# scienceguyrob/PulsarFeatureExtractor

Measured on AMD Instinct MI355X. Metric: candidates/sec (8-feature path, 128-bin), higher is better.
Workload: dtype u8->int64/f64; 1 GPU; config 2: 10000000 synthetic candidates per GPU, 128-bin profile + 128-bin DM, 8 Lyon moment features (pfe_lyon8_u8); candidates_per_gpu=10000000, dm_bins=128, parallelism=candidate shards x1, no collective

## Files before the change

### pulsarfeatureextractor_amd/csrc/lyon8.hip

```cpp

#include "options.h"
#include "pfe_common.h"

namespace pfe {

typedef short short2v __attribute__((ext_vector_type(2)));
typedef unsigned short ushort2v __attribute__((ext_vector_type(2)));
typedef uint32_t u32x4 __attribute__((ext_vector_type(4)));
typedef double f64x2 __attribute__((ext_vector_type(2)));

struct Moments {
  double mean, m2, m3, m4;
};

__device__ __forceinline__ Moments moments_i64(long long n, long long T1, long long T2,
                                               long long T3, unsigned long long T4) {
  typedef unsigned long long u64;
  const u64 un = (u64)n, t1 = (u64)T1, t2 = (u64)T2, t3 = (u64)T3;
  const u64 n2 = un * un, n3 = n2 * un;
  const u64 t1s = t1 * t1;
  const long long N2 = (long long)(un * t2 - t1s);
  const long long N3 = (long long)(n2 * t3 - 3ull * un * t1 * t2 + 2ull * t1s * t1);
  const u64 N4 = n3 * T4 - 4ull * n2 * t1 * t3 + 6ull * un * t1s * t2 - 3ull * t1s * t1s;
  const double dn = (double)n;
  Moments m;
  m.mean = (double)(T1 + 128ll * n) / dn;
  m.m2 = (double)N2 / (dn * dn);
  m.m3 = (double)N3 / (dn * dn * dn);
  m.m4 = (double)N4 / ((dn * dn) * (dn * dn));
  return m;
}

__device__ __forceinline__ double i128_to_f64(__int128 v) {
  const bool neg = v < 0;
  unsigned __int128 u = neg ? (unsigned __int128)(-v) : (unsigned __int128)v;
  const uint64_t hi = (uint64_t)(u >> 64), lo = (uint64_t)u;
  double r = (double)hi * 18446744073709551616.0 + (double)lo;
  return neg ? -r : r;
}

__device__ __forceinline__ Moments moments_i128(long long n, long long T1, long long T2,
                                                long long T3, unsigned long long T4) {
  typedef __int128 i128;
  const i128 in = n, t1 = T1, t2 = T2, t3 = T3, t4 = (i128)T4;
  const i128 n2 = in * in, n3 = n2 * in;
  const i128 t1s = t1 * t1;
  const i128 N2 = in * t2 - t1s;
  const i128 N3 = n2 * t3 - 3 * in * t1 * t2 + 2 * t1s * t1;
  const i128 N4 = n3 * t4 - 4 * n2 * t1 * t3 + 6 * in * t1s * t2 - 3 * t1s * t1s;
  const double dn = (double)n;
  Moments m;
  m.mean = (double)(T1 + 128ll * n) / dn;
  m.m2 = i128_to_f64(N2) / (dn * dn);
  m.m3 = i128_to_f64(N3) / (dn * dn * dn);
  m.m4 = i128_to_f64(N4) / ((dn * dn) * (dn * dn));
  return m;
}

__device__ __forceinline__ bool zero_var(const Moments& m) {
  const double e = 2.220446049250313e-16 * m.mean;
  return m.m2 <= e * e;
}

__device__ __forceinline__ double stat_k(const Moments& m, int k) {
  if (k == 0) return m.mean;
  if (k == 1) return sqrt(m.m2);
  if (zero_var(m)) return __builtin_nan("");
  if (k == 2) return m.m3 / (m.m2 * sqrt(m.m2));
  return m.m4 / (m.m2 * m.m2) - 3.0;
}

struct Acc2 {
  uint32_t s1, s2;
  int t3;
  uint64_t t4;
};

__device__ __forceinline__ void acc2_dword(uint32_t x, Acc2& a, uint32_t& t4a) {
  a.s1 = __builtin_amdgcn_udot4(x, 0x01010101u, a.s1, false);
  a.s2 = __builtin_amdgcn_udot4(x, x, a.s2, false);
  const uint32_t lo = __builtin_amdgcn_perm(0u, x, 0x0c020c00u);
  const uint32_t hi = __builtin_amdgcn_perm(0u, x, 0x0c030c01u);
  short2v ylo = __builtin_bit_cast(short2v, lo) - (short2v){128, 128};
  short2v yhi = __builtin_bit_cast(short2v, hi) - (short2v){128, 128};
  ushort2v qlo = __builtin_bit_cast(ushort2v, ylo) * __builtin_bit_cast(ushort2v, ylo);
  ushort2v qhi = __builtin_bit_cast(ushort2v, yhi) * __builtin_bit_cast(ushort2v, yhi);
  a.t3 = __builtin_amdgcn_sdot2(__builtin_bit_cast(short2v, qlo), ylo, a.t3, false);
  a.t3 = __builtin_amdgcn_sdot2(__builtin_bit_cast(short2v, qhi), yhi, a.t3, false);
  t4a = __builtin_amdgcn_udot2(qlo, qlo, t4a, false);
  t4a = __builtin_amdgcn_udot2(qhi, qhi, t4a, false);
}

__device__ __forceinline__ void acc2_x4(const u32x4 q, Acc2& a) {
  uint32_t u = 0, v = 0;
  acc2_dword(q.x, a, u);
  acc2_dword(q.y, a, u);
  acc2_dword(q.z, a, v);
  acc2_dword(q.w, a, v);
  a.t4 += (uint64_t)u + (uint64_t)v;
}

template <int G>
__device__ __forceinline__ void acc2_reduce(Acc2& a) {
  a.s1 = (uint32_t)group_sum_i32<G>((int)a.s1);
  a.s2 = (uint32_t)group_sum_i32<G>((int)a.s2);
  a.t3 = group_sum_i32<G>(a.t3);
  a.t4 = group_sum_u64<G>(a.t4);
}

template <int L>
__device__ __forceinline__ void stats4(const Acc2& a, double (&st)[4]) {
  constexpr double IN1 = 1.0 / L, IN2 = IN1 * IN1, IN3 = IN2 * IN1, IN4 = IN2 * IN2;
  const long long S1 = (long long)a.s1;
  const long long T1 = S1 - 128ll * L;
  const long long T2 = (long long)a.s2 - 256ll * S1 + 16384ll * L;
  const long long T3 = a.t3;
  typedef unsigned long long u64;
  const long long N2 = (long long)L * T2 - T1 * T1;
  const long long T1s = T1 * T1;
  const long long N3 = (long long)L * L * T3 - 3ll * L * T1 * T2 + 2ll * T1s * T1;
  const u64 N4 = (u64)L * L * L * a.t4 - 4ull * (u64)L * L * (u64)(T1 * T3) +
                 6ull * (u64)L * (u64)(T1s * T2) - 3ull * (u64)T1s * (u64)T1s;
  const double mean = (double)S1 * IN1;
  const double m2 = (double)N2 * IN2;
  const double m3 = (double)N3 * IN3;
  const double m4 = (double)N4 * IN4;
  const double sd = sqrt(m2);
  const double e = 2.220446049250313e-16 * mean;
  const bool zero = m2 <= e * e;
  st[0] = mean;
  st[1] = sd;
  st[2] = zero ? __builtin_nan("") : m3 / (m2 * sd);
  st[3] = zero ? __builtin_nan("") : m4 / (m2 * m2) - 3.0;
}

template <int L, int U>
__global__ __launch_bounds__(256) void lyon8_u8_fast3(const uint8_t* __restrict__ prof,
                                                      int64_t ps,
                                                      const uint8_t* __restrict__ dm,
                                                      int64_t ds, int64_t n,
                                                      double* __restrict__ out) {
  constexpr int LPC = L / 32;
  constexpr int CPW = 64 / LPC;
  constexpr int SPL = 8 / LPC;
  const int lane = threadIdx.x & 63;
  const int sub = lane % LPC;
  const int cw = lane / LPC;
  const int j0 = sub * SPL;
  const bool is_dm = j0 >= 4;
  const int64_t wave = ((int64_t)blockIdx.x * blockDim.x + threadIdx.x) >> 6;
  const int64_t step = (int64_t)CPW * U;
  const int64_t stride = (((int64_t)gridDim.x * blockDim.x) >> 6) * step;
  for (int64_t base = wave * step; base < n; base += stride) {
    u32x4 p[U][2], d[U][2];
#pragma unroll
    for (int u = 0; u < U; ++u) {
      int64_t c = base + u * CPW + cw;
      c = c < n ? c : n - 1;
      const u32x4* pp = reinterpret_cast<const u32x4*>(prof + c * ps + sub * 32);
      const u32x4* dp = reinterpret_cast<const u32x4*>(dm + c * ds + sub * 32);
      p[u][0] = __builtin_nontemporal_load(pp);
      p[u][1] = __builtin_nontemporal_load(pp + 1);
      d[u][0] = __builtin_nontemporal_load(dp);
      d[u][1] = __builtin_nontemporal_load(dp + 1);
    }
#pragma unroll
    for (int u = 0; u < U; ++u) {
      const int64_t c = base + u * CPW + cw;
      Acc2 sp = {0, 0, 0, 0}, sd = {0, 0, 0, 0};
      acc2_x4(p[u][0], sp);
      acc2_x4(p[u][1], sp);
      acc2_x4(d[u][0], sd);
      acc2_x4(d[u][1], sd);
      acc2_reduce<LPC>(sp);
      acc2_reduce<LPC>(sd);
      Acc2 s;
      s.s1 = is_dm ? sd.s1 : sp.s1;
      s.s2 = is_dm ? sd.s2 : sp.s2;
      s.t3 = is_dm ? sd.t3 : sp.t3;
      s.t4 = is_dm ? sd.t4 : sp.t4;
      double st[4];
      stats4<L>(s, st);
      if (c < n) {
        double* o = out + c * 8 + j0;
        if constexpr (SPL == 4) {
          __builtin_nontemporal_store((f64x2){st[0], st[1]}, reinterpret_cast<f64x2*>(o));
          __builtin_nontemporal_store((f64x2){st[2], st[3]}, reinterpret_cast<f64x2*>(o) + 1);
        } else if constexpr (SPL == 2) {
          const bool hi2 = (j0 & 3) != 0;
          __builtin_nontemporal_store((f64x2){hi2 ? st[2] : st[0], hi2 ? st[3] : st[1]},
                                      reinterpret_cast<f64x2*>(o));
        } else {
          const int k = j0 & 3;
          const double v = k == 0 ? st[0] : k == 1 ? st[1] : k == 2 ? st[2] : st[3];
          __builtin_nontemporal_store(v, o);
        }
      }
    }
  }
}

__global__ __launch_bounds__(256) void lyon8_u8_generic(const uint8_t* __restrict__ prof,
                                                        int64_t ps, int lp,
                                                        const uint8_t* __restrict__ dm,
                                                        int64_t ds, int ld, int64_t n,
                                                        double* __restrict__ out) {
  const int lane = threadIdx.x & 63;
  const int64_t wave = ((int64_t)blockIdx.x * blockDim.x + threadIdx.x) >> 6;
  const int64_t nwaves = ((int64_t)gridDim.x * blockDim.x) >> 6;
  for (int64_t w = wave; w < 2 * n; w += nwaves) {
    const int64_t c = w >> 1;
    const int row = (int)(w & 1);
    const uint8_t* p = row ? dm + c * ds : prof + c * ps;
    const int len = row ? ld : lp;
    long long t1 = 0, t2 = 0, t3 = 0;
    unsigned long long t4 = 0;
    for (int i = lane; i < len; i += 64) {
      const int y = (int)p[i] - 128;
      const int y2 = y * y;
      t1 += y;
      t2 += y2;
      t3 += (long long)(y2 * y);
      t4 += (unsigned long long)((uint32_t)y2 * (uint32_t)y2);
    }
    t1 = wave_sum_i64(t1);
    t2 = wave_sum_i64(t2);
    t3 = wave_sum_i64(t3);
    t4 = (unsigned long long)wave_sum_i64((long long)t4);
    if (lane < 4) {
      const Moments m = len <= 430 ? moments_i64(len, t1, t2, t3, t4)
                                   : moments_i128(len, t1, t2, t3, t4);
      out[c * 8 + row * 4 + lane] = stat_k(m, lane);
    }
  }
}

struct LongShape {
  int ld;
  int base[2];
  int m[2];
  int l[2];
  int lanes[2];
};

__device__ __forceinline__ double leaf_sumsq(const uint64_t (&w)[16], int nwords, double mean) {
  double r[8];
#pragma unroll
  for (int k = 0; k < 16; ++k) {
#pragma unroll
    for (int j = 0; j < 8; ++j) {
      const double d = (double)(uint32_t)((w[k] >> (8 * j)) & 0xFF) - mean;
      const double sq = k < nwords ? d * d : 0.0;
      if (k == 0)
        r[j] = sq;
      else
        r[j] += sq;
    }
  }
  return ((r[0] + r[1]) + (r[2] + r[3])) + ((r[4] + r[5]) + (r[6] + r[7]));
}

template <int LP>
__global__ __launch_bounds__(256) void lyon8_u8_long(const uint8_t* __restrict__ prof,
                                                     int64_t ps,
                                                     const uint8_t* __restrict__ dm,
                                                     int64_t ds, int64_t n,
                                                     double* __restrict__ out, LongShape sh) {
  constexpr int PL = LP / 16;
  const int lane = threadIdx.x & 63;
  const int h = lane >> 5, li = lane & 31;
  const int M = sh.m[h], L = sh.l[h];
  const bool has = li < sh.lanes[h];
  const int off0 = sh.base[h] + li * L * M;
  const int nw0 = has ? M / 8 : 0;
  const int nw1 = has && L == 2 ? M / 8 : 0;
  const int64_t wave = ((int64_t)blockIdx.x * blockDim.x + threadIdx.x) >> 6;
  const int64_t nwaves = ((int64_t)gridDim.x * blockDim.x) >> 6;
  for (int64_t c = wave; c < n; c += nwaves) {
    const uint8_t* drow = dm + c * ds;
    uint64_t w0[16], w1[16];
#pragma unroll
    for (int k = 0; k < 16; ++k) {
      const int a0 = k < nw0 ? off0 + 8 * k : 0;
      const int a1 = k < nw1 ? off0 + M + 8 * k : 0;
      w0[k] = __builtin_nontemporal_load(reinterpret_cast<const uint64_t*>(drow + a0));
      w1[k] = __builtin_nontemporal_load(reinterpret_cast<const uint64_t*>(drow + a1));
    }
    const int pl = lane < PL ? lane : 0;
    const u32x4 pq = __builtin_nontemporal_load(reinterpret_cast<const u32x4*>(prof + c * ps) + pl);
#pragma unroll
    for (int k = 0; k < 16; ++k) {
      if (k >= nw0) w0[k] = 0x8080808080808080ull;
      if (k >= nw1) w1[k] = 0x8080808080808080ull;
    }
    Acc2 sd = {0, 0, 0, 0};
#pragma unroll
    for (int k = 0; k < 16; k += 2) {
      acc2_x4((u32x4){(uint32_t)w0[k], (uint32_t)(w0[k] >> 32), (uint32_t)w0[k + 1],
                      (uint32_t)(w0[k + 1] >> 32)}, sd);
      acc2_x4((u32x4){(uint32_t)w1[k], (uint32_t)(w1[k] >> 32), (uint32_t)w1[k + 1],
                      (uint32_t)(w1[k + 1] >> 32)}, sd);
    }
    const int pad = 8 * (32 - nw0 - nw1);
    Acc2 sp = {0, 0, 0, 0};
    if (lane < PL) acc2_x4(pq, sp);
    const long long S1 = wave_sum_i64((long long)sd.s1 - 128ll * pad);
    const long long S2 = wave_sum_i64((long long)sd.s2 - 16384ll * pad);
    const long long T3 = wave_sum_i64((long long)sd.t3);
    const unsigned long long T4 = (unsigned long long)wave_sum_i64((long long)sd.t4);
    sp.s1 = (uint32_t)wave_sum_i64((long long)sp.s1);
    sp.s2 = (uint32_t)wave_sum_i64((long long)sp.s2);
    sp.t3 = (int)wave_sum_i64((long long)sp.t3);
    sp.t4 = (uint64_t)wave_sum_i64((long long)sp.t4);
    const double dn = (double)sh.ld;
    const double mean = (double)S1 / dn;
    const double ssq = wave_sum_f64(leaf_sumsq(w0, nw0, mean) + leaf_sumsq(w1, nw1, mean));
    if (lane < 8) {
      double v;
      if (lane < 4) {
        double st[4];
        stats4<LP>(sp, st);
        v = lane == 0 ? st[0] : lane == 1 ? st[1] : lane == 2 ? st[2] : st[3];
      } else {
        const long long T1 = S1 - 128ll * sh.ld;
        const long long T2 = S2 - 256ll * S1 + 16384ll * sh.ld;
        const Moments mo = moments_i128(sh.ld, T1, T2, T3, T4);
        const int k = lane - 4;
        v = k == 0 ? mean : k == 1 ? sqrt(ssq / dn) : stat_k(mo, k);
      }
      __builtin_nontemporal_store(v, out + c * 8 + lane);
    }
  }
}

constexpr int DPP_ROW_ROR8 = 0x128;

template <int CTRL>
__device__ __forceinline__ uint32_t dpp_u32(uint32_t v) {
  return (uint32_t)dpp_i32<CTRL>((int)v);
}

__device__ __forceinline__ uint32_t reduce_scatter8(const uint32_t (&v)[8], int t) {
  const bool b2 = t & 4, b1 = t & 2, b0 = t & 1;
  uint32_t a[4], b[2];
#pragma unroll
  for (int k = 0; k < 4; ++k)
    a[k] = (b2 ? v[k + 4] : v[k]) + dpp_u32<DPP_ROW_HALF_MIRROR>(b2 ? v[k] : v[k + 4]);
#pragma unroll
  for (int k = 0; k < 2; ++k)
    b[k] = (b1 ? a[k + 2] : a[k]) + dpp_u32<DPP_QUAD_XOR2>(b1 ? a[k] : a[k + 2]);
  return (b0 ? b[1] : b[0]) + dpp_u32<DPP_QUAD_XOR1>(b0 ? b[0] : b[1]);
}

__device__ __forceinline__ double swap16_sum(double v) {
  const long long x = __double_as_longlong(v);
  const unsigned lo = (unsigned)x, hi = (unsigned)((unsigned long long)x >> 32);
  const auto l = __builtin_amdgcn_permlane16_swap(lo, lo, false, false);
  const auto h = __builtin_amdgcn_permlane16_swap(hi, hi, false, false);
  return __longlong_as_double((long long)(((unsigned long long)h[0] << 32) | l[0])) +
         __longlong_as_double((long long)(((unsigned long long)h[1] << 32) | l[1]));
}
__device__ __forceinline__ double swap32_sum(double v) {
  const long long x = __double_as_longlong(v);
  const unsigned lo = (unsigned)x, hi = (unsigned)((unsigned long long)x >> 32);
  const auto l = __builtin_amdgcn_permlane32_swap(lo, lo, false, false);
  const auto h = __builtin_amdgcn_permlane32_swap(hi, hi, false, false);
  return __longlong_as_double((long long)(((unsigned long long)h[0] << 32) | l[0])) +
         __longlong_as_double((long long)(((unsigned long long)h[1] << 32) | l[1]));
}

__device__ __forceinline__ double leaf_tree64(double v) {
  v += dpp_f64<DPP_ROW_ROR8>(v);
  v = swap16_sum(v);
  v = swap32_sum(v);
  v += dpp_f64<DPP_QUAD_XOR1>(v);
  v += dpp_f64<DPP_QUAD_XOR2>(v);
  v += dpp_f64<DPP_ROW_HALF_MIRROR>(v);
  return v;
}

__device__ __forceinline__ void acc34_dword(uint32_t x, int& t3, uint32_t& t4a) {
  const uint32_t lo = __builtin_amdgcn_perm(0u, x, 0x0c020c00u);
  const uint32_t hi = __builtin_amdgcn_perm(0u, x, 0x0c030c01u);
  short2v ylo = __builtin_bit_cast(short2v, lo) - (short2v){128, 128};
  short2v yhi = __builtin_bit_cast(short2v, hi) - (short2v){128, 128};
  ushort2v qlo = __builtin_bit_cast(ushort2v, ylo) * __builtin_bit_cast(ushort2v, ylo);
  ushort2v qhi = __builtin_bit_cast(ushort2v, yhi) * __builtin_bit_cast(ushort2v, yhi);
  t3 = __builtin_amdgcn_sdot2(__builtin_bit_cast(short2v, qlo), ylo, t3, false);
  t3 = __builtin_amdgcn_sdot2(__builtin_bit_cast(short2v, qhi), yhi, t3, false);
  t4a = __builtin_amdgcn_udot2(qlo, qlo, t4a, false);
  t4a = __builtin_amdgcn_udot2(qhi, qhi, t4a, false);
}

template <int LP, int NI>
__global__ __launch_bounds__(256) void lyon8_u8_pow2(const uint8_t* __restrict__ prof,
                                                     int64_t ps,
                                                     const uint8_t* __restrict__ dm,
                                                     int64_t ds, int64_t n,
                                                     double* __restrict__ out) {
  static_assert(NI == 8 || NI == 16, "ld = 8192 or 16384");
  constexpr int PL = LP / 16;
  constexpr int K = NI == 16 ? 14 : 13;
  constexpr int LD = 1 << K;
  constexpr double SCALE = 1.0 / (double)(1ll << (2 * K));
  const int lane = threadIdx.x & 63;
  const int t = lane & 7;
  const int64_t wave = ((int64_t)blockIdx.x * blockDim.x + threadIdx.x) >> 6;
  const int64_t nwaves = ((int64_t)gridDim.x * blockDim.x) >> 6;
  for (int64_t c = wave; c < n; c += nwaves) {
    const u32x4* drow = reinterpret_cast<const u32x4*>(dm + c * ds) + lane;
    u32x4 q[NI];
#pragma unroll
    for (int i = 0; i < NI; ++i) q[i] = __builtin_nontemporal_load(drow + 64 * i);
    const int pl = lane < PL ? lane : 0;
    const u32x4 pq = __builtin_nontemporal_load(reinterpret_cast<const u32x4*>(prof + c * ps) + pl);
    uint32_t A[NI], B[NI];
    uint32_t s1 = 0, s2 = 0;
    int t3 = 0;
    uint64_t t4 = 0;
#pragma unroll
    for (int i = 0; i < NI; ++i) {
      uint32_t a = __builtin_amdgcn_udot4(q[i].x, 0x01010101u, 0u, false);
      a = __builtin_amdgcn_udot4(q[i].y, 0x01010101u, a, false);
      a = __builtin_amdgcn_udot4(q[i].z, 0x01010101u, a, false);
      a = __builtin_amdgcn_udot4(q[i].w, 0x01010101u, a, false);
      uint32_t b = __builtin_amdgcn_udot4(q[i].x, q[i].x, 0u, false);
      b = __builtin_amdgcn_udot4(q[i].y, q[i].y, b, false);
      b = __builtin_amdgcn_udot4(q[i].z, q[i].z, b, false);
      b = __builtin_amdgcn_udot4(q[i].w, q[i].w, b, false);
      A[i] = a;
      B[i] = b;
      s1 += a;
      s2 += b;
      uint32_t u = 0, v = 0;
      acc34_dword(q[i].x, t3, u);
      acc34_dword(q[i].y, t3, u);
      acc34_dword(q[i].z, t3, v);
      acc34_dword(q[i].w, t3, v);
      t4 += (uint64_t)u + (uint64_t)v;
    }
    Acc2 sp = {0, 0, 0, 0};
    if (lane < PL) acc2_x4(pq, sp);
    const long long S1 = wave_sum_i64((long long)s1);
    const long long S2 = wave_sum_i64((long long)s2);
    const long long T3 = wave_sum_i64((long long)t3);
    const unsigned long long T4 = (unsigned long long)wave_sum_i64((long long)t4);
    sp.s1 = (uint32_t)wave_sum_i64((long long)sp.s1);
    sp.s2 = (uint32_t)wave_sum_i64((long long)sp.s2);
    sp.t3 = (int)wave_sum_i64((long long)sp.t3);
    sp.t4 = (uint64_t)wave_sum_i64((long long)sp.t4);
    double ssq = 0.0;
#pragma unroll
    for (int s = 0; s < NI / 8; ++s) {
      uint32_t va[8], vb[8];
#pragma unroll
      for (int k = 0; k < 8; ++k) {
        va[k] = A[8 * s + k];
        vb[k] = B[8 * s + k];
      }
      const long long la = reduce_scatter8(va, t), lb = reduce_scatter8(vb, t);
      const long long v2k = (lb << (2 * K)) - ((2 * S1 * la) << K) + 128ll * S1 * S1;
      const double chunk = leaf_tree64((double)v2k * SCALE);
      ssq = s == 0 ? chunk : ssq + chunk;
    }
    if (lane < 8) {
      double v;
      if (lane < 4) {
        double st[4];
        stats4<LP>(sp, st);
        v = lane == 0 ? st[0] : lane == 1 ? st[1] : lane == 2 ? st[2] : st[3];
      } else {
        const double dn = (double)LD;
        const long long T1 = S1 - 128ll * LD;
        const long long T2 = S2 - 256ll * S1 + 16384ll * LD;
        const Moments mo = moments_i128(LD, T1, T2, T3, T4);
        const int k = lane - 4;
        v = k == 0 ? (double)S1 / dn : k == 1 ? sqrt(ssq / dn) : stat_k(mo, k);
      }
      __builtin_nontemporal_store(v, out + c * 8 + lane);
    }
  }
}

constexpr int L8_LDS_WAVE_BYTES = 64 * 144;

__device__ __forceinline__ void wave_lds_sync() {
  __builtin_amdgcn_fence(__ATOMIC_RELEASE, "wavefront");
  __builtin_amdgcn_wave_barrier();
  __builtin_amdgcn_fence(__ATOMIC_ACQUIRE, "wavefront");
}

__host__ __device__ constexpr int lds_leaf_stride(int m) { return m + ((m / 16) % 2 == 0 ? 16 : 32); }

template <int M>
__device__ __forceinline__ double leaf_sumsq_lds(const uint8_t* img, int leaf, double mean) {
  constexpr int S = lds_leaf_stride(M);
  uint64_t w[16];
// ... 452 lines not shown
      }
      double ssq = 0.0, a3 = 0.0, a4 = 0.0;
#pragma unroll
      for (int ch = 0; ch < NCH; ++ch) {
        if (ch > 0) dm_stage<NCH>(img, q, ch, lane, full_base, stab);
        wave_lds_sync();
        double l3, l4;
        double leaf;
        if (PAIRT)
          leaf = dm_leaf_tri_pair<FPM>(img, lane, nm, sc, z, l3, l4);
        else if (G == 3 && ch == NCH - 1)
          leaf = dm_leaf_tri<FPM>(img, lane, nm, sc, z, l3, l4);
        else if (G == 2 || G == 4 || G == 8) {
          if (ch == NCH - 1)
            leaf = dm_leaf<FPM, (G == 2 || G == 4 || G == 8) ? 8 / G : 8>(img + (lane / G) * DM_S,
                                                                       (8 / G) * (lane % G), nm, sc, z, nw_last, l3, l4);
          else
            leaf = dm_leaf<FPM>(img + lane * DM_S, 0, nm, sc, z, 16, l3, l4);
        }
        else
          leaf = dm_leaf<FPM>(img + lane * DM_S, 0, nm, sc, z, ch < NCH - 1 ? 16 : nw_last, l3, l4);
        if (ch == NCH - 1) {
          const bool in = leaf_last >= 0;
          leaf = in ? leaf : 0.0;
          l3 = in ? l3 : 0.0;
          l4 = in ? l4 : 0.0;
        }
        a3 += l3;
        a4 += l4;
        const double cs = PAIR ? half_sum_f64(leaf)
                          : (ch == NCH - 1 && G == 3) ? wave_sum_tri_split_f64(leaf)
                          : (ch == NCH - 1 && sh.tri) ? wave_sum_tri_f64(leaf) : wave_sum_f64(leaf);
        ssq = ch == 0 ? cs : ssq + cs;
        wave_lds_sync();
      }
      ssq = __builtin_ldexp(ssq, 102);
      if constexpr (FPM) {
        const double s3 = __builtin_ldexp(a3, 153), s4 = __builtin_ldexp(a4, 204);
        const uint64_t b3 = (uint64_t)__double_as_longlong(PAIR ? half_sum_f64(s3) : wave_sum_f64(s3));
        const uint64_t b4 = (uint64_t)__double_as_longlong(PAIR ? half_sum_f64(s4) : wave_sum_f64(s4));
        park_u32(kT3l, (uint32_t)b3);
        park_u32(kT3h, (uint32_t)(b3 >> 32));
        park_u32(kT4l, (uint32_t)b4);
        park_u32(kT4h, (uint32_t)(b4 >> 32));
      }
      if constexpr (PAIR) {
        const double va = lane_f64(ssq, 0), vb = lane_f64(ssq, 32);
        kssq = mine ? va : mine2 ? vb : kssq;
      } else {
        kssq = mine ? ssq : kssq;
      }
    }
    if (lane < cnt) {
      Acc2 sp = {0, 0, 0, 0};
      const u32x4* pr = reinterpret_cast<const u32x4*>(prof + (base + lane) * ps);
      for (int k = 0; k < ppl; ++k) acc2_x4(__builtin_nontemporal_load(pr + k), sp);
      const long long L = sh.lp;
      const long long S1p = (long long)sp.s1;
      const long long T1p = S1p - 128ll * L;
      const long long T2p = (long long)sp.s2 - 256ll * S1p + 16384ll * L;
      const long long T3p = (long long)sp.t3;
      const uint64_t T4p = sp.t4;
      const Moments mp = moments_i64(L, T1p, T2p, T3p, T4p);
      const double sdp = sqrt(mp.m2);
      const bool zp = zero_var(mp);
      const long long D = sh.ld;
      const long long S1 = (long long)kS1;
      const double dn = (double)D;
      Moments md;
      if constexpr (FPM) {
        md.mean = (double)S1 / dn;
        md.m3 = __longlong_as_double((long long)(((uint64_t)kT3h << 32) | kT3l)) / dn;
        md.m4 = __longlong_as_double((long long)(((uint64_t)kT4h << 32) | kT4l)) / dn;
      } else {
        const long long T1 = S1 - 128ll * D;
        const long long T2 = (long long)kS2 - 256ll * S1 + 16384ll * D;
        const long long T3 = (long long)(int)kT3h * 65536ll + (long long)kT3l;
        const uint64_t T4 = ((uint64_t)kT4h << 24) + (uint64_t)kT4l;
        md = moments_i128(D, T1, T2, T3, T4);
      }
      const double m2 = kssq / dn;
      const double e = 2.220446049250313e-16 * md.mean;
      const bool zd = m2 <= e * e;
      const double sdd = sqrt(m2);
      f64x2* o = reinterpret_cast<f64x2*>(out + (base + lane) * 8);
      __builtin_nontemporal_store((f64x2){mp.mean, sdp}, o);
      __builtin_nontemporal_store(
          (f64x2){zp ? __builtin_nan("") : mp.m3 / (mp.m2 * sdp),
                  zp ? __builtin_nan("") : mp.m4 / (mp.m2 * mp.m2) - 3.0}, o + 1);
      __builtin_nontemporal_store((f64x2){md.mean, sdd}, o + 2);
      __builtin_nontemporal_store(
          (f64x2){zd ? __builtin_nan("") : md.m3 / (m2 * sdd),
                  zd ? __builtin_nan("") : md.m4 / (m2 * m2) - 3.0}, o + 3);
    }
  }
}

__global__ __launch_bounds__(256) void lyon8_f64_generic(const double* __restrict__ prof,
                                                         int64_t ps, int lp,
                                                         const double* __restrict__ dm,
                                                         int64_t ds, int ld, int64_t n,
                                                         double* __restrict__ out) {
  const int lane = threadIdx.x & 63;
  const int64_t wave = ((int64_t)blockIdx.x * blockDim.x + threadIdx.x) >> 6;
  const int64_t nwaves = ((int64_t)gridDim.x * blockDim.x) >> 6;
  for (int64_t w = wave; w < 2 * n; w += nwaves) {
    const int64_t c = w >> 1;
    const int row = (int)(w & 1);
    const double* p = row ? dm + c * ds : prof + c * ps;
    const int len = row ? ld : lp;
    double s = 0.0;
    for (int i = lane; i < len; i += 64) s += p[i];
    s = wave_sum_f64(s);
    const double mean = s / (double)len;
    double a2 = 0.0, a3 = 0.0, a4 = 0.0;
    for (int i = lane; i < len; i += 64) {
      const double d = p[i] - mean;
      const double d2 = d * d;
      a2 += d2;
      a3 += d2 * d;
      a4 += d2 * d2;
    }
    a2 = wave_sum_f64(a2);
    a3 = wave_sum_f64(a3);
    a4 = wave_sum_f64(a4);
    if (lane < 4) {
      Moments m;
      m.mean = mean;
      m.m2 = a2 / (double)len;
      m.m3 = a3 / (double)len;
      m.m4 = a4 / (double)len;
      out[c * 8 + row * 4 + lane] = stat_k(m, lane);
    }
  }
}

}

namespace pfe {

static inline int grid_for(int64_t work_waves, int cap) {
  int64_t blocks = (work_waves + 3) / 4;
  if (blocks < 1) blocks = 1;
  if (blocks > cap) blocks = cap;
  return (int)blocks;
}

static bool perfect_chunk(int len, int& m, int& leaves) {
  leaves = 1;
  while (len > 128) {
    if (len % 16) return false;
    len /= 2;
    leaves *= 2;
  }
  m = len;
  return len > 64 && len % 8 == 0;
}

static bool place_half(LongShape& sh, int h, int base, int len) {
  int m, leaves;
  if (!perfect_chunk(len, m, leaves) || leaves > 64) return false;
  sh.base[h] = base;
  sh.m[h] = m;
  sh.l[h] = leaves > 32 ? 2 : 1;
  sh.lanes[h] = leaves > 32 ? 32 : leaves;
  return true;
}

static bool long_row_shape(int ld, LongShape& sh) {
  sh.ld = ld;
  if (ld <= 256) return false;
  if (ld <= 8192) {
    return ld % 16 == 0 && place_half(sh, 0, 0, ld / 2) && place_half(sh, 1, ld / 2, ld / 2);
  }
  if (ld <= 16384) return place_half(sh, 0, 0, 8192) && place_half(sh, 1, 8192, ld - 8192);
  return false;
}

static void np_leaves(int off, int n, int depth, int* start, int* len, int* dep, int& cnt, int cap) {
  if (n <= 128) {
    if (cnt < cap) {
      start[cnt] = off;
      len[cnt] = n;
      dep[cnt] = depth;
    }
    ++cnt;
    return;
  }
  int n2 = n / 2;
  n2 -= n2 % 8;
  np_leaves(off, n2, depth + 1, start, len, dep, cnt, cap);
  np_leaves(off + n2, n - n2, depth + 1, start, len, dep, cnt, cap);
}

static bool dm_shape(int lp, int ld, DmShape& sh, int& nch) {
  if (ld <= 256 || ld > 4 * 8192 || ld % 16) return false;
  nch = (ld + 8191) / 8192;
  const int len = ld - 8192 * (nch - 1);
  int start[DM_MAX_LEAVES], lens[DM_MAX_LEAVES], dep[DM_MAX_LEAVES], cnt = 0;
  np_leaves(0, len, 0, start, lens, dep, cnt, DM_MAX_LEAVES);
  if (cnt > DM_MAX_LEAVES) return false;
  bool tri = false;
  if (cnt == 48) {
    tri = true;
    for (int i = 0; i < cnt; ++i) {
      const int b = i / 3, k = i % 3;
      tri = tri && start[i] == 264 * b + (k == 0 ? 0 : k == 1 ? 128 : 192) &&
            lens[i] == (k == 0 ? 128 : k == 1 ? 64 : 72) && dep[i] == dep[0] + (k == 0 ? 0 : 1);
    }
    if (!tri) return false;
  } else {
    if ((cnt & (cnt - 1)) != 0) return false;
    for (int i = 0; i < cnt; ++i)
      if (dep[i] != dep[0] || lens[i] % 8 || lens[i] < 64 || lens[i] > 128) return false;
  }
  sh.lp = lp;
  sh.ld = ld;
  sh.len_last = len;
  sh.leaves_last = cnt;
  sh.tri = tri ? 1 : 0;
  for (int i = 0; i < cnt; ++i) sh.start[i] = (uint16_t)start[i];
  for (int i = cnt; i <= DM_MAX_LEAVES; ++i) sh.start[i] = (uint16_t)len;
  return true;
}

template <auto K>
static int resident_blocks() {
  static int cached[64] = {};
  int dev = 0;
  if (hipGetDevice(&dev) != hipSuccess || dev < 0 || dev >= 64) return 1024;
  if (cached[dev] > 0) return cached[dev];
  int per_cu = 0, cus = 0;
  if (hipOccupancyMaxActiveBlocksPerMultiprocessor(&per_cu, reinterpret_cast<const void*>(K), 256, 0) !=
          hipSuccess ||
      hipDeviceGetAttribute(&cus, hipDeviceAttributeMultiprocessorCount, dev) != hipSuccess) {
    (void)hipGetLastError();
    return 1024;
  }
  cached[dev] = (per_cu > 0 ? per_cu : 1) * (cus > 0 ? cus : 1);
  return cached[dev];
}

#ifndef PFE_DM_FPM_MAXCH
#define PFE_DM_FPM_MAXCH 4
#endif
template <int NCH, bool FPM, int G = 1>
static void launch_dm_kernel(const uint8_t* prof, int64_t ps, const uint8_t* dm, int64_t ds,
                             int64_t n, double* out, const DmShape& sh, hipStream_t st, int cap) {
  constexpr auto K = lyon8_u8_dm<NCH, FPM, G>;
  int64_t blocks = resident_blocks<K>();
  const int64_t need = (n + 3) / 4;
  if (blocks > need) blocks = need;
  if (blocks > cap) blocks = cap;
  if (blocks < 1) blocks = 1;
  hipLaunchKernelGGL(K, dim3((unsigned)blocks), dim3(256), 0, st, prof, ps, dm, ds, n, out, sh);
}

hipError_t launch_lyon8_u8(const uint8_t* prof, int64_t ps, int lp, const uint8_t* dm,
                           int64_t ds, int ld, int64_t n, double* out, hipStream_t st,
                           const Options& o) {
  if (n <= 0) return hipSuccess;
  const bool aligned = ((uintptr_t)prof % 16 == 0) && ((uintptr_t)dm % 16 == 0) &&
                       (ps % 16 == 0) && (ds % 16 == 0) && ((uintptr_t)out % 16 == 0);
  DmShape dsh{};
  int dnch = 0;
  if (o.lyon8_dm != 1 && aligned && (lp == 64 || lp == 128 || lp == 256) && ld != 8192 &&
      ld != 16384 && dm_shape(lp, ld, dsh, dnch)) {
    const int cap = o.lyon8_blocks;
    const int G = !o.lyon8_dm_split ? 1
                  : (dsh.tri && dnch == 1 && o.lyon8_dm_split == 1) ? 32
                  : dsh.tri ? 3
                  : (dnch == 1 && dsh.leaves_last > 16 && dsh.leaves_last <= 32 && o.lyon8_dm_split == 1) ? 16
                  : dsh.leaves_last <= 8 ? 8 : dsh.leaves_last <= 16 ? 4 : dsh.leaves_last <= 32 ? 2 : 1;
    if (o.lyon8_dm == 0 && dnch <= PFE_DM_FPM_MAXCH) {
#define PFE_DMK(C)                                                                   \
  switch (G) {                                                                       \
    case 8: launch_dm_kernel<C, true, 8>(prof, ps, dm, ds, n, out, dsh, st, cap); break; \
    case 4: launch_dm_kernel<C, true, 4>(prof, ps, dm, ds, n, out, dsh, st, cap); break; \
    case 2: launch_dm_kernel<C, true, 2>(prof, ps, dm, ds, n, out, dsh, st, cap); break; \
    case 3: launch_dm_kernel<C, true, 3>(prof, ps, dm, ds, n, out, dsh, st, cap); break; \
    case 16: if constexpr (C == 1) launch_dm_kernel<1, true, 16>(prof, ps, dm, ds, n, out, dsh, st, cap); break; \
    case 32: if constexpr (C == 1) launch_dm_kernel<1, true, 32>(prof, ps, dm, ds, n, out, dsh, st, cap); break; \
    default: launch_dm_kernel<C, true, 1>(prof, ps, dm, ds, n, out, dsh, st, cap); break; \
  }
      switch (dnch) {
        case 1: PFE_DMK(1) break;
        case 2: PFE_DMK(2) break;
#if PFE_DM_FPM_MAXCH > 2
        case 3: PFE_DMK(3) break;
        default: PFE_DMK(4) break;
#endif
      }
#undef PFE_DMK
    } else {
      switch (dnch) {
        case 1: launch_dm_kernel<1, false>(prof, ps, dm, ds, n, out, dsh, st, cap); break;
        case 2: launch_dm_kernel<2, false>(prof, ps, dm, ds, n, out, dsh, st, cap); break;
        case 3: launch_dm_kernel<3, false>(prof, ps, dm, ds, n, out, dsh, st, cap); break;
        default: launch_dm_kernel<4, false>(prof, ps, dm, ds, n, out, dsh, st, cap); break;
      }
    }
    return hipGetLastError();
  }
  if (aligned && lp == ld && (lp == 64 || lp == 128 || lp == 256)) {
    const int U = o.lyon8_burst;
    const int cpw = 64 / (lp / 32) * U;
    const int grid = grid_for((n + cpw - 1) / cpw, o.lyon8_blocks);
#define PFE_L8(LL, UU) \
  hipLaunchKernelGGL((lyon8_u8_fast3<LL, UU>), dim3(grid), dim3(256), 0, st, prof, ps, dm, ds, n, out)
#define PFE_L8U(LL)          \
  do {                       \
    if (U == 1)              \
      PFE_L8(LL, 1);         \
    else if (U == 4)         \
      PFE_L8(LL, 4);         \
    else                     \
      PFE_L8(LL, 2);         \
  } while (0)
    if (lp == 64)
      PFE_L8U(64);
    else if (lp == 128)
      PFE_L8U(128);
    else
      PFE_L8U(256);
#undef PFE_L8U
#undef PFE_L8
  } else if (aligned && (lp == 64 || lp == 128 || lp == 256) && (ld == 8192 || ld == 16384)) {
    const int grid = grid_for(n, o.lyon8_blocks);
#define PFE_L8P(LL, NN) \
  hipLaunchKernelGGL((lyon8_u8_pow2<LL, NN>), dim3(grid), dim3(256), 0, st, prof, ps, dm, ds, n, out)
    if (ld == 16384) {
      if (lp == 64)
        PFE_L8P(64, 16);
      else if (lp == 128)
        PFE_L8P(128, 16);
      else
        PFE_L8P(256, 16);
    } else {
      if (lp == 64)
        PFE_L8P(64, 8);
      else if (lp == 128)
        PFE_L8P(128, 8);
      else
        PFE_L8P(256, 8);
    }
#undef PFE_L8P
  } else if (int m1 = 0, l1 = 0; aligned && (lp == 64 || lp == 128 || lp == 256) && ld > 8192 &&
                                  ld < 16384 && ld % 16 == 0 && perfect_chunk(ld - 8192, m1, l1) &&
                                  m1 % 16 == 0) {
    const int grid = grid_for(n, o.lyon8_blocks);
#define PFE_L8S(LL, MM) \
  hipLaunchKernelGGL((lyon8_u8_lds<LL, MM>), dim3(grid), dim3(256), 0, st, prof, ps, dm, ds, n, out, ld)
#define PFE_L8SM(LL)          \
  do {                        \
    if (m1 == 80)             \
      PFE_L8S(LL, 80);        \
    else if (m1 == 96)        \
      PFE_L8S(LL, 96);        \
    else if (m1 == 112)       \
      PFE_L8S(LL, 112);       \
    else                      \
      PFE_L8S(LL, 128);       \
  } while (0)
    if (lp == 64)
      PFE_L8SM(64);
    else if (lp == 128)
      PFE_L8SM(128);
    else
      PFE_L8SM(256);
#undef PFE_L8SM
#undef PFE_L8S
  } else if (LongShape sh{}; aligned && (lp == 64 || lp == 128 || lp == 256) &&
                                long_row_shape(ld, sh)) {
    const int grid = grid_for(n, o.lyon8_blocks);
    if (lp == 64)
      hipLaunchKernelGGL(lyon8_u8_long<64>, dim3(grid), dim3(256), 0, st, prof, ps, dm, ds, n, out, sh);
    else if (lp == 128)
      hipLaunchKernelGGL(lyon8_u8_long<128>, dim3(grid), dim3(256), 0, st, prof, ps, dm, ds, n, out, sh);
    else
      hipLaunchKernelGGL(lyon8_u8_long<256>, dim3(grid), dim3(256), 0, st, prof, ps, dm, ds, n, out, sh);
  } else {
    const int grid = grid_for(2 * n, o.lyon8_blocks);
    hipLaunchKernelGGL(lyon8_u8_generic, dim3(grid), dim3(256), 0, st, prof, ps, lp, dm, ds, ld, n, out);
  }
  return hipGetLastError();
}

hipError_t launch_lyon8_f64(const double* prof, int64_t ps, int lp, const double* dm,
                            int64_t ds, int ld, int64_t n, double* out, hipStream_t st,
                            const Options& o) {
  if (n <= 0) return hipSuccess;
  const int grid = grid_for(2 * n, o.lyon8_blocks);
  hipLaunchKernelGGL(lyon8_f64_generic, dim3(grid), dim3(256), 0, st, prof, ps, lp, dm, ds, ld, n, out);
  return hipGetLastError();
}

}
```

Baseline: 18.16 billion candidates/sec.

## Narrow moment arithmetic and share stats4 work across duplicated lanes in lyon8 kernel

Reworks the per-candidate statistics in stats4 to use 32-bit and double arithmetic with power-of-two shifts in place of 64-bit multiplies. It also reassigns lanes so that lanes which previously computed the same profile/DM statistics redundantly now each handle a different candidate group, with DPP quad shuffles feeding the output stores. Addressing switches to 32-bit offsets from a per-iteration base pointer, and this is guarded by a new stride check on the host. The aim is to cut integer-multiply and redundant-ALU cost in a bandwidth-bound kernel, at the price of more complex lane mapping and narrower numeric range assumptions.

```diff
diff --git a/pulsarfeatureextractor_amd/csrc/lyon8.hip b/pulsarfeatureextractor_amd/csrc/lyon8.hip
--- a/pulsarfeatureextractor_amd/csrc/lyon8.hip
+++ b/pulsarfeatureextractor_amd/csrc/lyon8.hip
@@ -110,20 +110,27 @@
 
 template <int L>
 __device__ __forceinline__ void stats4(const Acc2& a, double (&st)[4]) {
+  static_assert(L <= 256 && (L & (L - 1)) == 0, "bounds of the narrow numerators");
+  constexpr int K = L == 256 ? 8 : L == 128 ? 7 : L == 64 ? 6 : L == 32 ? 5 : -1;
+  static_assert(K > 0 && (1 << K) == L, "L = 2^K");
   constexpr double IN1 = 1.0 / L, IN2 = IN1 * IN1, IN3 = IN2 * IN1, IN4 = IN2 * IN2;
-  const long long S1 = (long long)a.s1;
-  const long long T1 = S1 - 128ll * L;
-  const long long T2 = (long long)a.s2 - 256ll * S1 + 16384ll * L;
-  const long long T3 = a.t3;
   typedef unsigned long long u64;
-  const long long N2 = (long long)L * T2 - T1 * T1;
-  const long long T1s = T1 * T1;
-  const long long N3 = (long long)L * L * T3 - 3ll * L * T1 * T2 + 2ll * T1s * T1;
-  const u64 N4 = (u64)L * L * L * a.t4 - 4ull * (u64)L * L * (u64)(T1 * T3) +
-                 6ull * (u64)L * (u64)(T1s * T2) - 3ull * (u64)T1s * (u64)T1s;
-  const double mean = (double)S1 * IN1;
+  const int T1 = (int)a.s1 - 128 * L;
+  const int T2 = (int)(a.s2 - 256u * a.s1) + 16384 * L;
+  const int T3 = a.t3;
+  const int T1s = __mul24(T1, T1);
+  const int N2 = L * T2 - T1s;
+  const double d1 = (double)T1, d1s = (double)T1s;
+  const double N3 = ((double)T3 * (double)(L * L) - (d1 * (double)T2) * (double)(3 * L)) +
+                    (d1s * d1) * 2.0;
+  const uint32_t W = (uint32_t)(2 * L) * (uint32_t)T2 - (uint32_t)T1s;
+  u64 p13 = (u64)((long long)T1 * (long long)T3);
+  u64 pw = (u64)(uint32_t)T1s * (u64)W;
+  asm("" : "+v"(p13), "+v"(pw));
+  const u64 N4 = (a.t4 << (3 * K)) - (p13 << (2 * K + 2)) + ((pw << 1) + pw);
+  const double mean = (double)a.s1 * IN1;
   const double m2 = (double)N2 * IN2;
-  const double m3 = (double)N3 * IN3;
+  const double m3 = N3 * IN3;
   const double m4 = (double)N4 * IN4;
   const double sd = sqrt(m2);
   const double e = 2.220446049250313e-16 * mean;
@@ -134,6 +141,9 @@
   st[3] = zero ? __builtin_nan("") : m4 / (m2 * m2) - 3.0;
 }
 
+constexpr int DPP_QUAD_0011 = 0x50;
+constexpr int DPP_QUAD_2233 = 0xFA;
+
 template <int L, int U>
 __global__ __launch_bounds__(256) void lyon8_u8_fast3(const uint8_t* __restrict__ prof,
                                                       int64_t ps,
@@ -142,57 +152,109 @@
                                                       double* __restrict__ out) {
   constexpr int LPC = L / 32;
   constexpr int CPW = 64 / LPC;
-  constexpr int SPL = 8 / LPC;
+  constexpr int STEP = CPW * U;
+  constexpr int HL = LPC / 2;
+  constexpr int GPR = HL < U ? HL : U;
+  constexpr int ROUNDS = U / GPR;
+  constexpr int DUP = HL / GPR;
+  constexpr int SPL = 4 / DUP;
   const int lane = threadIdx.x & 63;
   const int sub = lane % LPC;
   const int cw = lane / LPC;
-  const int j0 = sub * SPL;
-  const bool is_dm = j0 >= 4;
-  const int64_t wave = ((int64_t)blockIdx.x * blockDim.x + threadIdx.x) >> 6;
-  const int64_t step = (int64_t)CPW * U;
-  const int64_t stride = (((int64_t)gridDim.x * blockDim.x) >> 6) * step;
-  for (int64_t base = wave * step; base < n; base += stride) {
+  const int row = sub & 1;
+  const int g = (sub >> 1) % GPR;
+  const int part = (sub >> 1) / GPR;
+  const int wib = __builtin_amdgcn_readfirstlane((int)(threadIdx.x >> 6));
+  const int wpb = (int)(blockDim.x >> 6);
+  const int64_t wave = (int64_t)blockIdx.x * wpb + wib;
+  const int64_t stride = (int64_t)gridDim.x * wpb * STEP;
+  const uint32_t ps32 = (uint32_t)ps, ds32 = (uint32_t)ds;
+  uint32_t prow[U], drow[U];
+#pragma unroll
+  for (int u = 0; u < U; ++u) {
+    prow[u] = (uint32_t)(u * CPW + cw) * ps32;
+    drow[u] = (uint32_t)(u * CPW + cw) * ds32;
+  }
+  const uint32_t lsub = (uint32_t)sub * 32u;
+  const uint32_t oofs = (uint32_t)((g * CPW + cw) * 64 + row * 32 + part * (SPL * 8));
+  for (int64_t base = wave * STEP; base < n; base += stride) {
+    const int64_t rem = n - base;
+    const int last = rem < STEP ? (int)rem - 1 : STEP - 1;
+    const uint8_t* pb = prof + base * ps;
+    const uint8_t* db = dm + base * ds;
+    const uint32_t pmax = (uint32_t)last * ps32, dmax = (uint32_t)last * ds32;
     u32x4 p[U][2], d[U][2];
 #pragma unroll
     for (int u = 0; u < U; ++u) {
-      int64_t c = base + u * CPW + cw;
-      c = c < n ? c : n - 1;
-      const u32x4* pp = reinterpret_cast<const u32x4*>(prof + c * ps + sub * 32);
-      const u32x4* dp = reinterpret_cast<const u32x4*>(dm + c * ds + sub * 32);
+      const uint32_t po = (prow[u] < pmax ? prow[u] : pmax) + lsub;
+      const uint32_t dq = (drow[u] < dmax ? drow[u] : dmax) + lsub;
+      const u32x4* pp = reinterpret_cast<const u32x4*>(pb + po);
+      const u32x4* dp = reinterpret_cast<const u32x4*>(db + dq);
       p[u][0] = __builtin_nontemporal_load(pp);
       p[u][1] = __builtin_nontemporal_load(pp + 1);
       d[u][0] = __builtin_nontemporal_load(dp);
       d[u][1] = __builtin_nontemporal_load(dp + 1);
     }
+    Acc2 sp[U], sd[U];
 #pragma unroll
     for (int u = 0; u < U; ++u) {
-      const int64_t c = base + u * CPW + cw;
-      Acc2 sp = {0, 0, 0, 0}, sd = {0, 0, 0, 0};
-      acc2_x4(p[u][0], sp);
-      acc2_x4(p[u][1], sp);
-      acc2_x4(d[u][0], sd);
-      acc2_x4(d[u][1], sd);
-      acc2_reduce<LPC>(sp);
-      acc2_reduce<LPC>(sd);
+      sp[u] = {0, 0, 0, 0};
+      sd[u] = {0, 0, 0, 0};
+      acc2_x4(p[u][0], sp[u]);
+      acc2_x4(p[u][1], sp[u]);
+      acc2_x4(d[u][0], sd[u]);
+      acc2_x4(d[u][1], sd[u]);
+      acc2_reduce<LPC>(sp[u]);
+      acc2_reduce<LPC>(sd[u]);
+    }
+    double* ob = out + base * 8;
+#pragma unroll
+    for (int r = 0; r < ROUNDS; ++r) {
+      const int u0 = r * GPR;
       Acc2 s;
-      s.s1 = is_dm ? sd.s1 : sp.s1;
-      s.s2 = is_dm ? sd.s2 : sp.s2;
-      s.t3 = is_dm ? sd.t3 : sp.t3;
-      s.t4 = is_dm ? sd.t4 : sp.t4;
+      s.s1 = row ? sd[u0].s1 : sp[u0].s1;
+      s.s2 = row ? sd[u0].s2 : sp[u0].s2;
+      s.t3 = row ? sd[u0].t3 : sp[u0].t3;
+      s.t4 = row ? sd[u0].t4 : sp[u0].t4;
+#pragma unroll
+      for (int k = 1; k < GPR; ++k) {
+        const bool mine = g == k;
+        const Acc2& a = sp[u0 + k];
+        const Acc2& b = sd[u0 + k];
+        s.s1 = mine ? (row ? b.s1 : a.s1) : s.s1;
+        s.s2 = mine ? (row ? b.s2 : a.s2) : s.s2;
+        s.t3 = mine ? (row ? b.t3 : a.t3) : s.t3;
+        s.t4 = mine ? (row ? b.t4 : a.t4) : s.t4;
+      }
       double st[4];
       stats4<L>(s, st);
-      if (c < n) {
-        double* o = out + c * 8 + j0;
+      if constexpr (SPL == 4 && LPC == 4) {
+        const bool hi = sub & 1;
+        double a[4], b[4];
+#pragma unroll
+        for (int k = 0; k < 4; ++k) {
+          a[k] = dpp_f64<DPP_QUAD_0011>(st[k]);
+          b[k] = dpp_f64<DPP_QUAD_2233>(st[k]);
+        }
+        const f64x2 v0 = {hi ? a[2] : a[0], hi ? a[3] : a[1]};
+        const f64x2 v1 = {hi ? b[2] : b[0], hi ? b[3] : b[1]};
+        char* o = reinterpret_cast<char*>(ob) + (uint32_t)(u0 * CPW * 64) +
+                  (uint32_t)(cw * 64 + sub * 16);
+        if (u0 * CPW + cw <= last) __builtin_nontemporal_store(v0, reinterpret_cast<f64x2*>(o));
+        if (u0 * CPW + CPW + cw <= last)
+          __builtin_nontemporal_store(v1, reinterpret_cast<f64x2*>(o + CPW * 64));
+      } else
+      if (u0 * CPW + g * CPW + cw <= last) {
+        double* o = reinterpret_cast<double*>(reinterpret_cast<char*>(ob) +
+                                              (uint32_t)(u0 * CPW * 64) + oofs);
         if constexpr (SPL == 4) {
           __builtin_nontemporal_store((f64x2){st[0], st[1]}, reinterpret_cast<f64x2*>(o));
           __builtin_nontemporal_store((f64x2){st[2], st[3]}, reinterpret_cast<f64x2*>(o) + 1);
         } else if constexpr (SPL == 2) {
-          const bool hi2 = (j0 & 3) != 0;
-          __builtin_nontemporal_store((f64x2){hi2 ? st[2] : st[0], hi2 ? st[3] : st[1]},
+          __builtin_nontemporal_store((f64x2){part ? st[2] : st[0], part ? st[3] : st[1]},
                                       reinterpret_cast<f64x2*>(o));
         } else {
-          const int k = j0 & 3;
-          const double v = k == 0 ? st[0] : k == 1 ? st[1] : k == 2 ? st[2] : st[3];
+          const double v = part == 0 ? st[0] : part == 1 ? st[1] : part == 2 ? st[2] : st[3];
           __builtin_nontemporal_store(v, o);
         }
       }
@@ -1251,7 +1313,8 @@
     }
     return hipGetLastError();
   }
-  if (aligned && lp == ld && (lp == 64 || lp == 128 || lp == 256)) {
+  const bool near = ps >= 0 && ds >= 0 && ps < (1 << 24) && ds < (1 << 24);
+  if (aligned && near && lp == ld && (lp == 64 || lp == 128 || lp == 256)) {
     const int U = o.lyon8_burst;
     const int cpw = 64 / (lp / 32) * U;
     const int grid = grid_for((n + cpw - 1) / cpw, o.lyon8_blocks);
```

Measured after the change: 18.45 billion candidates/sec, median of 6. +1.6%, better.
